# Rouslan/NTracer

Measured on AMD Instinct MI355X. Metric: Mrays/s (primary+shadow), 6-D hypercube @1920x1080, higher is better.
Workload: dtype f32

## Files before the change

ntracer_amd/csrc/nt_box.hpp:

```cpp
#pragma once
#include <type_traits>
#include "nt_pixel.hpp"

namespace {

__device__ __forceinline__ bool box_may_hit(int n, const float *dots, float sx, float sy, float sq) {
    const float osq = dots[0];
    const float ov = fmaf(-dots[2], sy, fmaf(dots[1], sx, dots[3]));
    const float rad2 = (float)n * (1.0f + NT_FUZZ) * (1.0f + NT_FUZZ) * 1.001f;
#ifdef NT_EXP_SKIP_SLABS
    return false;
#else
    return !((osq - rad2) * sq > ov * ov * 1.0001f);
#endif
}

__device__ __forceinline__ void box_background(float in, float &r, float &g, float &b) {
    if (in > 0.0f) { r = in; g = in; b = in; }
    else { r = 0.0f; g = -in; b = -in; }
}

template <int N>
__device__ __forceinline__ void box_color(const float (&o)[N], const float (&dir)[N], bool maybe, float &r, float &g, float &b) {
    bool done = false;
// ... 402 lines not shown
        return true;
    }
    emit_pixel(tg, pr, r, g, b);
    return true;
}

#ifndef NT_BOXROWS
#define NT_BOXROWS 8
#endif
template <int N>
__global__ __launch_bounds__(256) void box_kernel(NtCameraFixed cam, NtTarget tg) {
    const int tid = (int)threadIdx.x;
    float org[N], right[N], up[N], fwd[N], dir[N];
    load_camera<N>(cam, org, right, up, fwd);
    float margin = fabsf(org[0]);
#pragma unroll
    for (int j = 1; j < N; ++j) margin = fmaxf(margin, fabsf(org[j]));
    margin = NT_BOX_MARGIN * (1.0f + margin);
    float dots[4];
    if (cam.buf) {
        const float *dp = cam.dots + (size_t)blockIdx.z * 4;
        dots[0] = dp[0]; dots[1] = dp[1]; dots[2] = dp[2]; dots[3] = dp[3];
    } else {
        dots[0] = cam.odots[0]; dots[1] = cam.odots[1]; dots[2] = cam.odots[2]; dots[3] = cam.odots[3];
    }
    if (tg.colors_out) {
        const PixelRef pr = locate_pixel<64, 4>(tg, tid & 63, tid >> 6, tid);
        if (!pr.valid) return;
        const float sx = tg.fovI * ((float)pr.x - tg.half_w);
        const float sy = tg.fovI * ((float)pr.y - tg.half_h);
#pragma unroll
        for (int j = 0; j < N; ++j) dir[j] = (fwd[j] + right[j] * sx) - up[j] * sy;
        float sq = dir[0] * dir[0];
#pragma unroll
        for (int j = 1; j < N; ++j) sq = sq + dir[j] * dir[j];
        box_pixel<N, false>(tg, pr, org, dir, sq, dots, sx, sy, margin);
        return;
    }
    constexpr int R = NT_BOXROWS;
    const int row0 = ((int)blockIdx.y * 4 + __builtin_amdgcn_readfirstlane(tid >> 6)) * R;
    const int x = (int)blockIdx.x * 64 + (tid & 63);
    if (x >= tg.width) return;
    const float sx = tg.fovI * ((float)x - tg.half_w);
    float base[N];
#pragma unroll
    for (int j = 0; j < N; ++j) base[j] = fwd[j] + right[j] * sx;
    uint32_t live = ~0u;
    if (tg.cull) {
        if (row0 >= tg.row_count) return;
        const uint32_t *cp = tg.cull + ((size_t)blockIdx.z * tg.row_count + row0) * tg.cull_words + (blockIdx.x >> 3);
        live = 0u;
#pragma unroll
        for (int rr = 0; rr < R; ++rr) live |= (((cp[rr * tg.cull_words] >> (4 * (blockIdx.x & 7))) & 15u) != 0u ? 1u : 0u) << rr;
    }
    for (int rr = 0; rr < R; ++rr) {
        const int row = row0 + rr;
        if (row >= tg.row_count) return;
        const bool rowhit = (live >> rr) & 1u;
        const int orow = tg.row_begin + row;
        const int y = nt_image_row(tg, orow);
        if (y >= tg.height) continue;
        PixelRef pr;
        pr.x = x;
        pr.y = y;
        pr.offset = (long long)blockIdx.z * tg.frame_stride + (long long)(tg.compact ? orow : y) * tg.pitch + (long long)x * tg.bpp;
        pr.hit_index = 0;
        pr.valid = true;
        const float sy = tg.fovI * ((float)y - tg.half_h);
#pragma unroll
        for (int j = 0; j < N; ++j) dir[j] = base[j] - up[j] * sy;
        float sq = dir[0] * dir[0];
#pragma unroll
        for (int j = 1; j < N; ++j) sq = sq + dir[j] * dir[j];
        box_pixel<N, false>(tg, pr, org, dir, sq, dots, sx, sy, margin, rowhit);
    }
}

template <int N, int SPLIT>
__global__ __launch_bounds__(256) void box_redo_kernel(NtCameraFixed cam, NtTarget tg) {
    const int tid = (int)threadIdx.x;
    const int wv = __builtin_amdgcn_readfirstlane(tid >> 6);
    static_assert(SPLIT == 1 || SPLIT == 2 || SPLIT == 4, "waves per redo word");
    const int row = (int)blockIdx.y * (4 / SPLIT) + wv / SPLIT;
    if (row >= tg.row_count) return;
    uint32_t *word = tg.redo + ((size_t)blockIdx.z * tg.row_count + row) * tg.redo_words + blockIdx.x;
    const uint32_t mine = (SPLIT == 1 ? 0xffffffffu : SPLIT == 2 ? 0x55555555u : 0x11111111u) << (wv % SPLIT);
    uint32_t todo = *word & mine;
    if (todo == 0u) return;
    if ((tid & 63) == 0) {
        if (SPLIT > 1) atomicAnd(word, ~mine);
        else *word = 0u;
    }
    float org[N], right[N], up[N], fwd[N], dir[N];
    load_camera<N>(cam, org, right, up, fwd);
    float margin = fabsf(org[0]);
#pragma unroll
    for (int j = 1; j < N; ++j) margin = fmaxf(margin, fabsf(org[j]));
    margin = NT_BOX_MARGIN * (1.0f + margin);
    float dots[4];
    if (cam.buf) {
        const float *dp = cam.dots + (size_t)blockIdx.z * 4;
        dots[0] = dp[0]; dots[1] = dp[1]; dots[2] = dp[2]; dots[3] = dp[3];
    } else {
        dots[0] = cam.odots[0]; dots[1] = cam.odots[1]; dots[2] = cam.odots[2]; dots[3] = cam.odots[3];
    }
    const int orow = tg.row_begin + row;
    const int y = nt_image_row(tg, orow);
    if (y >= tg.height) return;
    const float sy = tg.fovI * ((float)y - tg.half_h);
    while (todo != 0u) {
        const int bit = __builtin_ctz(todo);
        todo &= todo - 1u;
        int x = ((int)blockIdx.x * 32 + bit) * 64 + (tid & 63);
        x = x < tg.width ? x : tg.width - 1;
        PixelRef pr;
        pr.x = x;
        pr.y = y;
        pr.offset = (long long)blockIdx.z * tg.frame_stride + (long long)(tg.compact ? orow : y) * tg.pitch + (long long)x * tg.bpp;
        pr.hit_index = 0;
        pr.valid = true;
        const float sx = tg.fovI * ((float)x - tg.half_w);
#pragma unroll
        for (int j = 0; j < N; ++j) dir[j] = (fwd[j] + right[j] * sx) - up[j] * sy;
        float sq = dir[0] * dir[0];
#pragma unroll
        for (int j = 1; j < N; ++j) sq = sq + dir[j] * dir[j];
        box_pixel<N, true, false, true>(tg, pr, org, dir, sq, dots, sx, sy, margin);
    }
}

template <int N, bool SETS = false>
__device__ __forceinline__ unsigned long long box_stretch_code2(const float (&org)[N], const float (&right)[N], const float (&up)[N],
                                                                const float (&fwd)[N], const NtTarget &tg, int y, int col) {
    uint32_t sets_value = 0u;
    uint32_t *const sets = SETS ? &sets_value : nullptr;
    uint32_t code = 0u;
    float omax = fabsf(org[0]);
#pragma unroll
    for (int j = 1; j < N; ++j) omax = fmaxf(omax, fabsf(org[j]));
    const float m = NT_BOX_MARGIN * (1.0f + omax);
    const float h = 1.0f + 2.0f * m + 1e-3f;
    const float sxc = tg.fovI * (((float)(col * 64) + 31.5f) - tg.half_w);
    const float sy = tg.fovI * ((float)y - tg.half_h);
    const float spread = 32.0f * tg.fovI;
    float tlo = 0.0f, thi = INFINITY;
    float vc[N], g[N];
    float tn = -INFINITY, tn2 = -INFINITY, vK = 0.0f, gK = 0.0f, oK = 0.0f;
    int K = 0;
#pragma unroll
    for (int j = 0; j < N; ++j) {
        vc[j] = (fwd[j] + right[j] * sxc) - up[j] * sy;
        g[j] = fmaf(spread, fabsf(right[j]), 1e-6f);
        const float pa = vc[j] + g[j], qa = -h - org[j];
        const float pb = vc[j] - g[j], qb = h - org[j];
        const float ra = qa * __builtin_amdgcn_rcpf(pa), rb = qb * __builtin_amdgcn_rcpf(pb);
        const bool ap = pa >= 0.0f, bp = pb >= 0.0f;
        const float lo_a = ap ? ra : -INFINITY, hi_a = ap ? INFINITY : ra;
        const float hi_b = bp ? rb : INFINITY, lo_b = bp ? -INFINITY : rb;
        tlo = nt_vmax3(tlo, lo_a, lo_b);
        thi = nt_vmin3(thi, hi_a, hi_b);
    }
    if (!(tlo > thi)) {
        code = 15u;
#pragma unroll
        for (int j = 0; j < N; ++j) {
            const float nr = ((vc[j] < 0.0f ? 1.0f : -1.0f) - org[j]) * __builtin_amdgcn_rcpf(vc[j]);
            tn2 = nt_vmed3(tn, tn2, nr);
            const bool later = nr > tn;
            vK = later ? vc[j] : vK;
            gK = later ? g[j] : gK;
            oK = later ? org[j] : oK;
            K = later ? j : K;
            tn = nt_vmax(tn, nr);
        }
        const float vKa = vK - gK, vKb = vK + gK;
        if (K < 13 && vKa * vKb > 0.0f) {
            const float num = (vK < 0.0f ? 1.0f : -1.0f) - oK;
            const float t1 = num * __builtin_amdgcn_rcpf(vKa), t2 = num * __builtin_amdgcn_rcpf(vKb);
            const float t_lo = nt_vmin(t1, t2) * (1.0f - 1e-6f), t_hi = nt_vmax(t1, t2) * (1.0f + 1e-6f);
            const float rK = m * __builtin_amdgcn_rcpf(fabsf(vK) - gK) * (1.0f + 1e-6f);
            bool ok = t_lo > 1e-3f && t_hi < 1e30f;
#pragma unroll
            for (int j = 0; j < N; ++j) {
                const float va = vc[j] - g[j], vb = vc[j] + g[j];
                const float pmax = org[j] + nt_vmax(vb * t_lo, vb * t_hi);
                const float pmin = org[j] + nt_vmin(va * t_lo, va * t_hi);
                const float lim = (1.0f - m - 1e-4f) - (fabsf(vc[j]) + g[j]) * rK;
                ok = ok && (j == K || (pmax <= lim && pmin >= -lim));
            }
            if (ok) code = (uint32_t)K + 1u;
        }
        if (code == 15u && !((tn - tn2) * fabsf(vK) > m)) code = 14u;
        if (code >= 14u) {
            if (sets != nullptr && N <= 10) {
                auto range = [&](int j, float &A, float &B, float &vabs) {
                    const float va = vc[j] - g[j], vb = vc[j] + g[j];
                    const float num = (vc[j] < 0.0f ? 1.0f : -1.0f) - org[j];
                    const float e1 = num * __builtin_amdgcn_rcpf(va), e2 = num * __builtin_amdgcn_rcpf(vb);
                    const float lo = nt_vmin(e1, e2), hi = nt_vmax(e1, e2);
                    const bool same = va * vb > 0.0f;
                    A = same ? lo - fabsf(lo) * 1e-6f : -INFINITY;
                    B = same ? hi + fabsf(hi) * 1e-6f : INFINITY;
                    vabs = same ? fabsf(vc[j]) - g[j] : 0.0f;
                };
                float rA[N], rB[N], rV[N];
                float TN = -INFINITY, TH = -INFINITY;
#pragma unroll
                for (int j = 0; j < N; ++j) {
                    range(j, rA[j], rB[j], rV[j]);
                    TN = nt_vmax(TN, rA[j]);
                    TH = nt_vmax(TH, rB[j]);
                }
                float vmin = INFINITY;
#pragma unroll
                for (int j = 0; j < N; ++j) vmin = rB[j] >= TN ? nt_vmin(vmin, rV[j]) : vmin;
                const float M = m * __builtin_amdgcn_rcpf(vmin) * (1.0f + 1e-5f);
                uint32_t T = 0u, C = 0u;
                float t_lo = INFINITY;
                const float t_hi = TH;
#pragma unroll
                for (int j = 0; j < N; ++j) {
                    const bool inT = rB[j] >= TN - M;
                    T |= inT ? 1u << j : 0u;
                    t_lo = inT ? nt_vmin(t_lo, rA[j]) : t_lo;
                }
#pragma unroll
                for (int j = 0; j < N; ++j) {
                    const float va = vc[j] - g[j], vb = vc[j] + g[j];
                    const float pmax = org[j] + nt_vmax(vb * t_lo, vb * t_hi);
                    const float pmin = org[j] + nt_vmin(va * t_lo, va * t_hi);
                    const float lim = 1.0f - m - 1e-4f;
                    const bool inC = ((T >> j) & 1u) != 0u || !(pmax <= lim && pmin >= -lim);
                    C |= inC ? 1u << j : 0u;
                }
                const bool valid = vmin > 0.0f && t_lo > 1e-3f && t_hi < 1e30f;
                *sets = valid ? (0x80000000u | (C << 10) | T) : 0u;
            }
        }
    }
    return (unsigned long long)code | ((unsigned long long)sets_value << 32);
}
template <int N>
__device__ __forceinline__ uint32_t box_stretch_code(const float (&org)[N], const float (&right)[N], const float (&up)[N], const float (&fwd)[N],
                                                     const NtTarget &tg, int y, int col) {
    return (uint32_t)box_stretch_code2<N, false>(org, right, up, fwd, tg, y, col);
}

template <int N>
__global__ __launch_bounds__(256) void box_cull_kernel(NtCameraFixed cam, NtTarget tg, uint32_t *out, int ncols) {
    float org[N], right[N], up[N], fwd[N];
    load_camera<N>(cam, org, right, up, fwd);
    const int word = (int)blockIdx.x, row = (int)blockIdx.y * 8 + (int)(threadIdx.x >> 5);
    const int col = word * 32 + (int)(threadIdx.x & 31);
    uint32_t code = 0u;
    if (row < tg.row_count && col < ncols) {
        const int orow = tg.row_begin + row;
        const int y = nt_image_row(tg, orow);
        code = box_stretch_code<N>(org, right, up, fwd, tg, y, col);
    }
    uint32_t packed = code << (4 * (threadIdx.x & 7));
    packed |= (uint32_t)__shfl_xor((int)packed, 1, 64);
    packed |= (uint32_t)__shfl_xor((int)packed, 2, 64);
    packed |= (uint32_t)__shfl_xor((int)packed, 4, 64);
    if (row < tg.row_count && (threadIdx.x & 7) == 0) out[((size_t)blockIdx.z * tg.row_count + row) * tg.cull_words + (col >> 3)] = packed;
}

#ifdef NT_EXP_NOSTORE
#define NT_EXP_STORE_IF if (tg.width < 0)
#else
#define NT_EXP_STORE_IF
#endif
#ifndef NT_TILE_OCC
#define NT_TILE_OCC
#endif
#ifndef NT_BOX_PIN_UP
#define NT_BOX_PIN_UP 1
#endif
#ifndef NT_BOX_LEAN_GROUPS_MAX_N
#define NT_BOX_LEAN_GROUPS_MAX_N 20
#endif
__device__ __forceinline__ bool guard_clear(float t) { return fabsf(__builtin_amdgcn_fractf(t) - 0.5f) > fmaf(t, 0x1p-18f, 0x1p-18f); }
__device__ __forceinline__ float lean_quotient(float d, float sy, float uu, float m2bu, float bb) {
    return fabsf(d) * __builtin_amdgcn_rsqf(fmaf(sy, fmaf(sy, uu, m2bu), bb));
}
template <int N>
__device__ __forceinline__ void pick_component(uint32_t K, const float (&base)[N], const float (&upv)[N], float &bK, float &uK) {
    bK = base[0];
    uK = upv[0];
#pragma unroll
    for (int j = 1; j < N; ++j) {
        bK = K == (uint32_t)j ? base[j] : bK;
        uK = K == (uint32_t)j ? upv[j] : uK;
    }
}
template <int N>
__device__ __forceinline__ float row_dir(const float (&base)[N], const float (&upv)[N], float sy, float (&dir)[N]) {
#pragma unroll
    for (int j = 0; j < N; ++j) dir[j] = base[j] - upv[j] * sy;
    float sq = dir[0] * dir[0];
#pragma unroll
    for (int j = 1; j < N; ++j) sq = sq + dir[j] * dir[j];
    return sq;
}
template <int N, bool F32, int ROWS, int WAVES>
__global__ __launch_bounds__(64 * WAVES) NT_TILE_OCC void box_tile_kernel(NtCameraFixed cam, NtTarget tg) {
    static_assert(ROWS == 8 || ROWS == 16 || ROWS == 32 || ROWS == 64, "sixteen row codes to a qword, one to four qwords a wave");
    static_assert(WAVES >= 1 && WAVES <= 4 && WAVES * ROWS <= 64, "the codes of a tile are the work of one wave, a row per lane");
    constexpr int R = ROWS;
    __shared__ uint32_t s_code[64];
    __shared__ unsigned long long s_rows[4];
    constexpr bool ALLIN = F32 || N <= NT_BOX_INLINE_MAX_N;
    constexpr bool SETS_LDS = ALLIN && N <= NT_BOX_SETS_MAX_N;
    __shared__ uint32_t s_sets[SETS_LDS ? 64 : 1];
    __shared__ int s_abort;
    const int tid = (int)threadIdx.x;
    const int lane = tid & 63;
    const int wv = __builtin_amdgcn_readfirstlane(tid >> 6);
#ifdef NT_EXP_TRACE
    const unsigned long long trace_t0 = wall_clock64();
    unsigned trace_rows = 0u;
    unsigned long long trace_t1 = 0ull;
#endif
    const unsigned nframes = gridDim.z - (unsigned)tg.lead_frames;
    unsigned frame = blockIdx.z;
    if (tg.lead_frames > 0) {
        const unsigned cols = gridDim.x, q = cols / 4u;
        const bool middle = blockIdx.x >= q && blockIdx.x < cols - q;
        if (!middle) frame -= (unsigned)tg.lead_frames;
        if (frame >= nframes) return;
    }
    float org[N], right[N], up[N], fwd[N], dir[N];
    load_camera<N>(cam, frame, org, right, up, fwd);
    float margin = fabsf(org[0]);
#pragma unroll
    for (int j = 1; j < N; ++j) margin = fmaxf(margin, fabsf(org[j]));
    margin = NT_BOX_MARGIN * (1.0f + margin);
    float dots[4];
    if (cam.buf) {
        const float *dp = cam.dots + (size_t)frame * 4;
        dots[0] = dp[0]; dots[1] = dp[1]; dots[2] = dp[2]; dots[3] = dp[3];
    } else {
        dots[0] = cam.odots[0]; dots[1] = cam.odots[1]; dots[2] = cam.odots[2]; dots[3] = cam.odots[3];
    }
    const int tile_row0 = (int)blockIdx.y * WAVES * R;
    if (wv == (int)((blockIdx.x + blockIdx.y + frame) % (unsigned)WAVES)) {
        if (tg.abort_word != nullptr) {
            const bool ab = nt_aborted(tg);
            if (WAVES == 1) { if (ab) return; }
            else if (lane == 0) s_abort = ab ? 1 : 0;
        }
        uint32_t code = 0u;
        uint32_t row_sets = 0u;
        const int trow = tg.row_il > 0 ? ((int)blockIdx.y * WAVES + lane / R) + tg.row_il * (lane % R) : tile_row0 + lane;
        if (lane < WAVES * R && trow < tg.row_count) {
            const int orow = tg.row_begin + trow;
            const int y = nt_image_row(tg, orow);
            if (y < tg.height) {
                const unsigned long long cs = box_stretch_code2<N, (N <= NT_BOX_SETS_MAX_N)>(org, right, up, fwd, tg, y, (int)blockIdx.x);
                code = (uint32_t)cs;
                row_sets = (uint32_t)(cs >> 32);
            }
        }
        if (SETS_LDS) s_sets[lane] = row_sets;
        {
            const unsigned long long m0 = __builtin_amdgcn_ballot_w64(code == 0u), m1 = __builtin_amdgcn_ballot_w64(code >= 1u && code <= 13u),
                                     m2 = __builtin_amdgcn_ballot_w64(code == 15u), m3 = __builtin_amdgcn_ballot_w64(code == 14u);
            if (lane == 0) {
                s_rows[0] = m0;
                s_rows[1] = m1;
                s_rows[2] = m2;
                s_rows[3] = m3;
            }
        }
        uint32_t packed = code << (4 * (lane & 7));
        packed |= (uint32_t)__shfl_xor((int)packed, 1, 64);
        packed |= (uint32_t)__shfl_xor((int)packed, 2, 64);
        packed |= (uint32_t)__shfl_xor((int)packed, 4, 64);
        if ((lane & 7) == 0) {
            const int grp = lane >> 3;
            const int slot = R == 8 ? 2 * grp : grp;
            s_code[slot] = packed;
            if (R == 8) s_code[slot + 1] = 0u;
        }
    }
    __syncthreads();
    if (WAVES > 1 && tg.abort_word != nullptr && s_abort != 0) return;
#ifdef NT_EXP_TRACE
    trace_t1 = wall_clock64();
#endif
    constexpr int HALVES = R >= 32 ? R / 16 : 1;
    const int wrow0 = tile_row0 + wv * R;
    const int il = tg.row_il;
    const int wfirst = il > 0 ? (int)blockIdx.y * WAVES + wv : wrow0;
    if (wfirst < tg.row_count) {
        typedef uint32_t nt_u32x4 __attribute__((ext_vector_type(4)));
        typedef __attribute__((address_space(4))) const nt_u32x4 *nt_rowtab;
        typedef uint32_t nt_u32x16 __attribute__((ext_vector_type(16), aligned(16)));
        typedef __attribute__((address_space(4))) const nt_u32x16 *nt_rowtab4;
        constexpr bool GROUPS = !F32 && N <= NT_BOX_LEAN_GROUPS_MAX_N;
        uint8_t *const frame_base = tg.dest + (long long)frame * tg.frame_stride;
#define NT_ROW_LOAD(rr)                     \
        const nt_u32x4 row_e = tab[(rr)];   \
        const float sy = __uint_as_float(row_e.x)
#define NT_ROW_OFF() ((long long)(((unsigned long long)row_e.w << 32) | row_e.z) + (long long)frame * tg.frame_stride)
#define NT_ROW_PTR() uniform_ptr(frame_base + (long long)(((unsigned long long)row_e.w << 32) | row_e.z))
#define NT_GROUP_PTR(k) uniform_ptr(frame_base + (long long)(((unsigned long long)grp_e[4 * (k) + 3] << 32) | grp_e[4 * (k) + 2]))
#define NT_LANE_OFF() ({ asm volatile("" : "+v"(xoff)); xoff; })
#define NT_CLEAR_BIT(mask, bit) asm("s_bitset0_b32 %0, %1" : "+s"(mask) : "s"(bit))
#define NT_SET_BIT(mask, bit) asm("s_bitset1_b32 %0, %1" : "+s"(mask) : "s"(bit))
        int x = (int)blockIdx.x * 64 + lane;
        x = x < tg.width ? x : tg.width - 1;
        uint32_t xoff = (uint32_t)x * (uint32_t)tg.bpp;
        const float sx = tg.fovI * ((float)x - tg.half_w);
        float base[N];
#pragma unroll
        for (int j = 0; j < N; ++j) base[j] = fwd[j] + right[j] * sx;
        float upv[N];
#pragma unroll
        for (int j = 0; j < N; ++j) {
            upv[j] = up[j];
            if (NT_BOX_PIN_UP || F32 || j == 0) asm volatile("" : "+v"(upv[j]));
        }
        float bb = 0.0f, bu = 0.0f, uu = 0.0f;
        bool fastsq = true;
        if (!F32) {
#pragma unroll
            for (int j = 0; j < N; ++j) {
                bb = fmaf(base[j], base[j], bb);
                bu = fmaf(base[j], up[j], bu);
                uu = fmaf(up[j], up[j], uu);
            }
            fastsq = __builtin_amdgcn_ballot_w64(!(bu * bu <= bb * uu * 0.0625f)) == 0ull;
        }
        const float maxv = (float)tg.plain_maxval;
        const float inv_maxv2 = 1.0f / (maxv * maxv);
        const float m2bu = (-2.0f * bu) * inv_maxv2;
        bb = bb * inv_maxv2;
        uu = uu * inv_maxv2;
        auto rows_of = [&](int k) {
            const unsigned long long m = s_rows[k];
            return (((unsigned long long)(uint32_t)__builtin_amdgcn_readfirstlane((int)(uint32_t)(m >> 32)) << 32) |
                    (uint32_t)__builtin_amdgcn_readfirstlane((int)(uint32_t)m)) >> (wv * R);
        };
        const unsigned long long rows_culled = rows_of(0), rows_face = rows_of(1), rows_rays = rows_of(2), rows_tie = rows_of(3);
        const int lrow = il > 0 ? wfirst + il * lane : wrow0 + lane;
        const int ly = nt_image_row(tg, tg.row_begin + lrow);
        const unsigned long long rows_valid = __builtin_amdgcn_ballot_w64(lane < R && lrow < tg.row_count && ly < tg.height);
#pragma unroll 1
        for (int half = 0; half < HALVES; ++half) {
        const int row0 = wrow0 + 16 * half;
        const int hfirst = il > 0 ? wfirst + il * 16 * half : row0;
        if (hfirst >= tg.row_count) break;
        uint32_t redo_bits = 0u;
        const int cw = (R >= 32 ? (R / 8) * wv + 2 * half : 2 * wv);
        unsigned long long rowcodes = ((unsigned long long)(uint32_t)__builtin_amdgcn_readfirstlane((int)s_code[cw + 1]) << 32) |
                                      (uint32_t)__builtin_amdgcn_readfirstlane((int)s_code[cw]);
        const uint32_t valid = HALVES > 1 ? (uint32_t)(rows_valid >> (16 * half)) & 0xffffu : (uint32_t)rows_valid;
        const nt_rowtab tab = (nt_rowtab)tg.rowtab + (il > 0 ? row0 : tg.row_begin + row0);
        uint32_t quick = (uint32_t)(rows_culled >> (16 * half)) & valid, inner = (uint32_t)(rows_face >> (16 * half)) & valid;
        uint32_t todo = (uint32_t)((ALLIN ? rows_rays | rows_tie : rows_rays) >> (16 * half)) & valid;
        if (!ALLIN) redo_bits = (uint32_t)(rows_tie >> (16 * half)) & valid;
#ifdef NT_EXP_TRACE
        trace_rows += (unsigned)__builtin_popcount(quick) | ((unsigned)__builtin_popcount(inner) << 8) |
                      ((unsigned)__builtin_popcount((uint32_t)(rows_rays >> (16 * half)) & valid) << 16) |
                      ((unsigned)__builtin_popcount((uint32_t)(rows_tie >> (16 * half)) & valid) << 24);
#endif
        if (!F32) {
            if (!fastsq) {
                todo |= quick | inner;
                quick = 0u;
                inner = 0u;
            }
            auto lean_rows = [&](auto sel8) {
            constexpr bool SEL8 = decltype(sel8)::value;
            auto put_quick = [&](nt_gptr out, float t, float d0) {
                if (SEL8) {
                    const uint32_t q = __float_as_uint(t + 8388608.0f);
                    NT_EXP_STORE_IF NT_G32(out) = __builtin_amdgcn_perm(d0 > 0.0f ? q : 0u, q, tg.plain_sel);
                    return;
                }
                uint32_t q = (uint32_t)(t + 0.5f);
                q = q < tg.plain_maxval ? q : tg.plain_maxval;
                const uint32_t w = (d0 > 0.0f ? q : 0u) * tg.plain_mul[0] + q * (tg.plain_mul[1] + tg.plain_mul[2]);
                NT_EXP_STORE_IF NT_G32(out) = tg.reversed ? w : bswap32(w);
            };
            auto put_face = [&](nt_gptr out, float t, float th) {
                if (SEL8) {
                    NT_EXP_STORE_IF NT_G32(out) = __builtin_amdgcn_perm(__float_as_uint(t + 8388608.0f), __float_as_uint(th + 8388608.0f), tg.plain_sel);
                    return;
                }
                uint32_t qr = (uint32_t)(t + 0.5f), qgb = (uint32_t)(th + 0.5f);
                qr = qr < tg.plain_maxval ? qr : tg.plain_maxval;
                qgb = qgb < tg.plain_maxval ? qgb : tg.plain_maxval;
                const uint32_t w = qr * tg.plain_mul[0] + qgb * (tg.plain_mul[1] + tg.plain_mul[2]);
                NT_EXP_STORE_IF NT_G32(out) = tg.reversed ? w : bswap32(w);
            };
            auto full_groups = [](uint32_t mask) { return mask & (mask >> 1) & (mask >> 2) & (mask >> 3) & 0x1111u; };
            auto lean_group = [&](int g, auto row, auto put) {
                const nt_u32x16 grp_e = *(nt_rowtab4)(tab + g);
                float a[4], b[4];
                unsigned long long fail[4];
#pragma unroll
                for (int k = 0; k < 4; ++k) fail[k] = __builtin_amdgcn_ballot_w64(!row(__uint_as_float(grp_e[4 * k]), a[k], b[k]));
                if (__builtin_expect(((fail[0] | fail[1]) | (fail[2] | fail[3])) == 0ull, 1)) {
                    const uint32_t xo = NT_LANE_OFF();
                    put(NT_GROUP_PTR(0) + xo, a[0], b[0]);
                    put(NT_GROUP_PTR(1) + xo, a[1], b[1]);
                    put(NT_GROUP_PTR(2) + xo, a[2], b[2]);
                    put(NT_GROUP_PTR(3) + xo, a[3], b[3]);
                } else {
                    todo |= ((fail[0] != 0ull ? 1u : 0u) | (fail[1] != 0ull ? 2u : 0u) | (fail[2] != 0ull ? 4u : 0u) | (fail[3] != 0ull ? 8u : 0u)) << g;
#pragma unroll
                    for (int k = 0; k < 4; ++k) {
                        if (fail[k] == 0ull) {
                            uint32_t xo = xoff;
                            asm volatile("" : "+v"(xo));
                            put(NT_GROUP_PTR(k) + xo, a[k], b[k]);
                        }
                    }
                }
            };
            auto culled_row = [&](float sy, float &t, float &d0) {
                d0 = base[0] - upv[0] * sy;
                t = lean_quotient(d0, sy, uu, m2bu, bb);
                return guard_clear(t);
            };
            auto face_row = [&](float bK, float uK, float sy, float &t, float &th) {
                const float dK = bK - uK * sy;
                t = lean_quotient(dK, sy, uu, m2bu, bb);
                th = t * 0.5f;
                return guard_clear(t) && guard_clear(th);
            };
            if (GROUPS) {
                uint32_t full = full_groups(quick);
                quick &= ~(full * 15u);
                while (full != 0u) {
                    const int g = __builtin_ctz(full);
                    NT_CLEAR_BIT(full, g);
                    lean_group(g, culled_row, put_quick);
                }
            }
            uint32_t quick_stored = 0u;
            for (uint32_t rest = quick; rest != 0u;) {
                const int rr = __builtin_ctz(rest);
                NT_CLEAR_BIT(rest, rr);
                NT_ROW_LOAD(rr);
                float t, d0;
                if (__builtin_expect(__builtin_amdgcn_ballot_w64(!culled_row(sy, t, d0)) == 0ull, 1)) {
                    put_quick(NT_ROW_PTR() + NT_LANE_OFF(), t, d0);
                    NT_SET_BIT(quick_stored, rr);
                }
            }
            todo |= quick & ~quick_stored;
            uint32_t K0 = 0u;
            float bK0 = base[0], uK0 = upv[0];
            if (inner != 0u) {
                K0 = ((uint32_t)(rowcodes >> (4 * __builtin_ctz(inner))) & 15u) - 1u;
                pick_component<N>(K0, base, upv, bK0, uK0);
            }
            if (GROUPS) {
                uint32_t full = full_groups(inner);
                const uint32_t same = (K0 + 1u) * 0x1111u;
                while (full != 0u) {
                    const int g = __builtin_ctz(full);
                    NT_CLEAR_BIT(full, g);
                    if (((uint32_t)(rowcodes >> (4 * g)) & 0xffffu) != same) continue;
                    inner &= ~(15u << g);
                    lean_group(g, [&](float sy, float &t, float &th) { return face_row(bK0, uK0, sy, t, th); }, put_face);
                }
            }
            uint32_t inner_stored = 0u;
            for (uint32_t rest = inner; rest != 0u;) {
                const int rr = __builtin_ctz(rest);
                NT_CLEAR_BIT(rest, rr);
                const uint32_t K = ((uint32_t)(rowcodes >> (4 * rr)) & 15u) - 1u;
                NT_ROW_LOAD(rr);
                float bK = bK0, uK = uK0;
                if (K != K0) pick_component<N>(K, base, upv, bK, uK);
                float t, th;
                if (__builtin_expect(__builtin_amdgcn_ballot_w64(!face_row(bK, uK, sy, t, th)) == 0ull, 1)) {
                    put_face(NT_ROW_PTR() + NT_LANE_OFF(), t, th);
                    NT_SET_BIT(inner_stored, rr);
                }
            }
            todo |= inner & ~inner_stored;
            };
            if (tg.plain_sel != 0u) lean_rows(std::true_type{});
            else lean_rows(std::false_type{});
        } else {
            while (quick != 0u) {
                const int rr = __builtin_ctz(quick);
                quick &= quick - 1u;
                NT_ROW_LOAD(rr);
                const float sq = row_dir<N>(base, upv, sy, dir);
                const float in = dir[0] / sqrt_wave(sq);
                float r, gb, b_;
                box_background(in, r, gb, b_);
                emit_f32x3_at(tg, NT_ROW_PTR() + NT_LANE_OFF(), r, gb);
            }
            uint32_t K0 = 0u;
            float bK0 = base[0], uK0 = upv[0];
            if (inner != 0u) {
                K0 = ((uint32_t)(rowcodes >> (4 * __builtin_ctz(inner))) & 15u) - 1u;
                pick_component<N>(K0, base, upv, bK0, uK0);
            }
            while (inner != 0u) {
                const int rr = __builtin_ctz(inner);
                inner &= inner - 1u;
                const uint32_t K = ((uint32_t)(rowcodes >> (4 * rr)) & 15u) - 1u;
                NT_ROW_LOAD(rr);
                const float sq = row_dir<N>(base, upv, sy, dir);
                float bK = bK0, uK = uK0;
                if (K != K0) pick_component<N>(K, base, upv, bK, uK);
                const float xk = bK - uK * sy;
                const float shade = fabsf(xk / sqrt_wave(sq));
                emit_f32x3_at(tg, NT_ROW_PTR() + NT_LANE_OFF(), shade * 1.0f, shade * 0.5f);
            }
        }
        while (todo != 0u) {
            const int rr = __builtin_ctz(todo);
            todo &= todo - 1u;
            const bool rowhit = ((uint32_t)(rowcodes >> (4 * rr)) & 15u) != 0u;
            NT_ROW_LOAD(rr);
            PixelRef pr;
            pr.x = x;
            pr.y = 0;
            pr.offset = NT_ROW_OFF() + (long long)xoff;
            pr.hit_index = 0;
            pr.valid = true;
            const float sq = row_dir<N>(base, upv, sy, dir);
            const int rcode = (int)((uint32_t)(rowcodes >> (4 * rr)) & 15u);
            if (ALLIN) {
                uint32_t sets = 0u;
                if (SETS_LDS) sets = (uint32_t)__builtin_amdgcn_readfirstlane((int)s_sets[wv * R + 16 * half + rr]);
                box_pixel<N, !F32, false, false, F32>(tg, pr, org, dir, sq, dots, sx, sy, margin, rowhit, rcode >= 1 && rcode <= 13 ? rcode - 1 : -1, sets,
                                                       rcode == 14);
            } else if (!box_pixel<N, true, true, false, false>(tg, pr, org, dir, sq, dots, sx, sy, margin, rowhit, rcode >= 1 && rcode <= 13 ? rcode - 1 : -1)) {
                redo_bits |= 1u << rr;
            }
        }
        if (!ALLIN && lane == 0) {
            while (redo_bits != 0u) {
                const int rr = __builtin_ctz(redo_bits);
                redo_bits &= redo_bits - 1u;
                const int mrow = il > 0 ? hfirst + il * rr : row0 + rr;
                atomicOr(tg.redo + ((size_t)frame * tg.row_count + mrow) * tg.redo_words + (blockIdx.x >> 5), 1u << (blockIdx.x & 31));
            }
        }
        }
    }
#ifdef NT_EXP_TRACE
    if (lane == 0) {
        unsigned long long *tr = reinterpret_cast<unsigned long long *>(tg.dest + (long long)nframes * tg.frame_stride) +
                                 ((((size_t)frame * gridDim.y + blockIdx.y) * gridDim.x + blockIdx.x) * WAVES + wv) * 4;
        tr[0] = trace_t0;
        tr[1] = wall_clock64();
        tr[2] = (unsigned long long)__builtin_amdgcn_s_getreg(4 | (31 << 11)) | ((unsigned long long)__builtin_amdgcn_s_getreg(20 | (31 << 11)) << 32);
        tr[3] = (unsigned long long)trace_rows | ((trace_t1 - trace_t0) << 32);
    }
#endif
#undef NT_ROW_LOAD
#undef NT_ROW_OFF
#undef NT_ROW_PTR
#undef NT_GROUP_PTR
#undef NT_LANE_OFF
#undef NT_CLEAR_BIT
#undef NT_SET_BIT
}

template <int N>
int launch_box_fixed(const NtLaunchInfo &li, const NtCamera &cam, const NtTarget &tg_in) {
    NtCameraFixed cf;
    cf.buf = cam.buf;
    cf.dots = cam.dots;
    for (int k = 0; k < 4; ++k) cf.odots[k] = cam.odots[k];
    cf.n = N;
    for (int k = 0; k < 4 * N; ++k) cf.inl[k] = cam.inl[k];
    NtTarget tg = tg_in;
    dim3 grid;
    grid_for(tg, 64, tg.colors_out ? 4 : 4 * NT_BOXROWS, li.nframes, grid);
    tg.cull = nullptr;
    tg.redo = nullptr;
    tg.cull_words = 0;
    tg.redo_words = 0;
    const bool fmt_rgb = tg.plain_bits != 0u && tg.plain_bits <= 10u && tg.bpp == 4 && tg.aligned4;
    const bool fmt_f32 = tg.plain_f32[0] >= 0 && tg.bpp == 12 && tg.aligned4;
    if (li.cull_buf && tg.rowtab && !tg.colors_out && (fmt_rgb || fmt_f32) && li.cull_clean) {
        hipStream_t st = (hipStream_t)li.stream;
        NtBoxTileGeom geom;
        geom.rows = li.tile_rows;
        geom.waves = li.tile_waves;
        const bool r64 = geom.rows == 64, r16 = geom.rows == 16;
        const int wpb = geom.waves;
        const int tile_rows = geom.rows * geom.waves;
        dim3 tgrid((unsigned)((tg.width + 63) / 64), (unsigned)((tg.row_count + tile_rows - 1) / tile_rows), (unsigned)li.nframes);
        tg.redo_words = ((tg.width + 63) / 64 + 31) / 32;
        tg.redo = li.cull_buf;
        tg.lead_frames = li.nframes >= 8 ? (li.nframes < 96 ? li.nframes : 96) : 0;
        if (tg.row_il > 0) tg.lead_frames = li.nframes >= 32 ? 16 : 0;
        if ((long long)li.nframes + tg.lead_frames > 65535) tg.lead_frames = 0;
        tgrid.z += (unsigned)tg.lead_frames;
        if (fmt_rgb) {
            if (r64) hipLaunchKernelGGL((box_tile_kernel<N, false, 64, 1>), tgrid, dim3(64), 0, st, cf, tg);
            else if (r16 && wpb == 3) hipLaunchKernelGGL((box_tile_kernel<N, false, 16, 3>), tgrid, dim3(192), 0, st, cf, tg);
            else if (r16) hipLaunchKernelGGL((box_tile_kernel<N, false, 16, 4>), tgrid, dim3(256), 0, st, cf, tg);
            else hipLaunchKernelGGL((box_tile_kernel<N, false, 8, 4>), tgrid, dim3(256), 0, st, cf, tg);
            if constexpr (N > NT_BOX_INLINE_MAX_N) {
                const long long rwords = (long long)tg.row_count * li.nframes * tg.redo_words;
                const int split = rwords < 48 * 1024 ? 2 : 1;
                const int rpb = 4 / split;
                const dim3 rgrid((unsigned)tg.redo_words, (unsigned)((tg.row_count + rpb - 1) / rpb), (unsigned)li.nframes);
                if (split == 2) hipLaunchKernelGGL((box_redo_kernel<N, 2>), rgrid, dim3(256), 0, st, cf, tg);
                else hipLaunchKernelGGL((box_redo_kernel<N, 1>), rgrid, dim3(256), 0, st, cf, tg);
            }
        } else {
            if (r64) hipLaunchKernelGGL((box_tile_kernel<N, true, 64, 1>), tgrid, dim3(64), 0, st, cf, tg);
            else if (r16 && wpb == 3) hipLaunchKernelGGL((box_tile_kernel<N, true, 16, 3>), tgrid, dim3(192), 0, st, cf, tg);
            else if (r16) hipLaunchKernelGGL((box_tile_kernel<N, true, 16, 4>), tgrid, dim3(256), 0, st, cf, tg);
            else hipLaunchKernelGGL((box_tile_kernel<N, true, 8, 4>), tgrid, dim3(256), 0, st, cf, tg);
        }
        return 0;
    }
    if (li.cull_buf && !tg.colors_out) {
        const int ncols = (tg.width + 63) / 64;
        const int words = (ncols + 31) / 32;
        tg.cull_words = 4 * words;
        hipLaunchKernelGGL(box_cull_kernel<N>, dim3((unsigned)words, (unsigned)((tg.row_count + 7) / 8), (unsigned)li.nframes), dim3(256), 0,
                           (hipStream_t)li.stream, cf, tg, li.cull_buf, ncols);
        tg.cull = li.cull_buf;
    }
    hipLaunchKernelGGL(box_kernel<N>, grid, dim3(256), 0, (hipStream_t)li.stream, cf, tg);
    return 0;
}

}
```

Before: 1.023 million.

## Keep per-row codes in registers for single-wave tiles and group face rows by axis

For single-wave blocks (ROWS=64), per-row codes and set bits now stay in a lane register and are read with readlane and ballots, instead of going through LDS with a block barrier. All 64 rows are handled in one pass using 64-bit masks. Face rows are grouped by hit axis, so each component is picked once per group and same-axis rows can use the grouped lean path. The cost is extra readlane traffic and 64-bit mask arithmetic. ROWS=32 configurations are no longer allowed.

After: 1.102 million, median of 6. 1.08x the previous value.

```diff
diff --git a/ntracer_amd/csrc/nt_box.hpp b/ntracer_amd/csrc/nt_box.hpp
--- a/ntracer_amd/csrc/nt_box.hpp
+++ b/ntracer_amd/csrc/nt_box.hpp
@@ -728,17 +728,34 @@
     for (int j = 1; j < N; ++j) sq = sq + dir[j] * dir[j];
     return sq;
 }
+#ifndef NT_BOX_PASS_ROWS
+#define NT_BOX_PASS_ROWS 64
+#endif
+__device__ __forceinline__ int nt_low_bit(uint32_t m) { return __builtin_ctz(m); }
+__device__ __forceinline__ int nt_low_bit(unsigned long long m) { return __builtin_ctzll(m); }
+__device__ __forceinline__ int nt_count_bits(uint32_t m) { return __builtin_popcount(m); }
+__device__ __forceinline__ int nt_count_bits(unsigned long long m) { return __builtin_popcountll(m); }
+__device__ __forceinline__ void nt_clear_bit(uint32_t &m, int bit) { asm("s_bitset0_b32 %0, %1" : "+s"(m) : "s"(bit)); }
+__device__ __forceinline__ void nt_clear_bit(unsigned long long &m, int bit) { asm("s_bitset0_b64 %0, %1" : "+s"(m) : "s"(bit)); }
+__device__ __forceinline__ void nt_set_bit(uint32_t &m, int bit) { asm("s_bitset1_b32 %0, %1" : "+s"(m) : "s"(bit)); }
+__device__ __forceinline__ void nt_set_bit(unsigned long long &m, int bit) { asm("s_bitset1_b64 %0, %1" : "+s"(m) : "s"(bit)); }
+__device__ __forceinline__ void nt_drop_low_bit(uint32_t &m, int) { m &= m - 1u; }
+__device__ __forceinline__ void nt_drop_low_bit(unsigned long long &m, int bit) { nt_clear_bit(m, bit); }
 template <int N, bool F32, int ROWS, int WAVES>
 __global__ __launch_bounds__(64 * WAVES) NT_TILE_OCC void box_tile_kernel(NtCameraFixed cam, NtTarget tg) {
-    static_assert(ROWS == 8 || ROWS == 16 || ROWS == 32 || ROWS == 64, "sixteen row codes to a qword, one to four qwords a wave");
+    static_assert(ROWS == 8 || ROWS == 16 || ROWS == 64, "a wave's rows: a qword of sixteen codes in LDS or fewer, or one row a lane");
     static_assert(WAVES >= 1 && WAVES <= 4 && WAVES * ROWS <= 64, "the codes of a tile are the work of one wave, a row per lane");
+    static_assert(WAVES == 1 ? ROWS == 64 : ROWS <= 16, "one wave a block renders the 64 rows whose codes it worked out itself");
     constexpr int R = ROWS;
-    __shared__ uint32_t s_code[64];
-    __shared__ unsigned long long s_rows[4];
+    constexpr bool REG = WAVES == 1;
+    constexpr int LDS_N = REG ? 1 : 64;
+    __shared__ uint32_t s_code[LDS_N];
+    __shared__ unsigned long long s_rows[REG ? 1 : 4];
     constexpr bool ALLIN = F32 || N <= NT_BOX_INLINE_MAX_N;
     constexpr bool SETS_LDS = ALLIN && N <= NT_BOX_SETS_MAX_N;
-    __shared__ uint32_t s_sets[SETS_LDS ? 64 : 1];
+    __shared__ uint32_t s_sets[SETS_LDS ? LDS_N : 1];
     __shared__ int s_abort;
+    uint32_t lane_cs = 0u;
     const int tid = (int)threadIdx.x;
     const int lane = tid & 63;
     const int wv = __builtin_amdgcn_readfirstlane(tid >> 6);
@@ -769,11 +786,11 @@
         dots[0] = cam.odots[0]; dots[1] = cam.odots[1]; dots[2] = cam.odots[2]; dots[3] = cam.odots[3];
     }
     const int tile_row0 = (int)blockIdx.y * WAVES * R;
-    if (wv == (int)((blockIdx.x + blockIdx.y + frame) % (unsigned)WAVES)) {
+    if (REG || wv == (int)((blockIdx.x + blockIdx.y + frame) % (unsigned)WAVES)) {
         if (tg.abort_word != nullptr) {
             const bool ab = nt_aborted(tg);
-            if (WAVES == 1) { if (ab) return; }
-            else if (lane == 0) s_abort = ab ? 1 : 0;
+            if constexpr (REG) { if (ab) return; }
+            else { if (lane == 0) s_abort = ab ? 1 : 0; }
         }
         uint32_t code = 0u;
         uint32_t row_sets = 0u;
@@ -787,34 +804,42 @@
                 row_sets = (uint32_t)(cs >> 32);
             }
         }
-        if (SETS_LDS) s_sets[lane] = row_sets;
-        {
-            const unsigned long long m0 = __builtin_amdgcn_ballot_w64(code == 0u), m1 = __builtin_amdgcn_ballot_w64(code >= 1u && code <= 13u),
-                                     m2 = __builtin_amdgcn_ballot_w64(code == 15u), m3 = __builtin_amdgcn_ballot_w64(code == 14u);
-            if (lane == 0) {
-                s_rows[0] = m0;
-                s_rows[1] = m1;
-                s_rows[2] = m2;
-                s_rows[3] = m3;
-            }
-        }
-        uint32_t packed = code << (4 * (lane & 7));
-        packed |= (uint32_t)__shfl_xor((int)packed, 1, 64);
-        packed |= (uint32_t)__shfl_xor((int)packed, 2, 64);
-        packed |= (uint32_t)__shfl_xor((int)packed, 4, 64);
-        if ((lane & 7) == 0) {
-            const int grp = lane >> 3;
-            const int slot = R == 8 ? 2 * grp : grp;
-            s_code[slot] = packed;
-            if (R == 8) s_code[slot + 1] = 0u;
-        }
-    }
-    __syncthreads();
-    if (WAVES > 1 && tg.abort_word != nullptr && s_abort != 0) return;
+        if constexpr (REG) {
+            lane_cs = (SETS_LDS ? row_sets & 0x800fffffu : 0u) | (code << 20);
+        } else {
+            if (SETS_LDS) s_sets[lane] = row_sets;
+            {
+                const unsigned long long m0 = __builtin_amdgcn_ballot_w64(code == 0u), m1 = __builtin_amdgcn_ballot_w64(code >= 1u && code <= 13u),
+                                         m2 = __builtin_amdgcn_ballot_w64(code == 15u), m3 = __builtin_amdgcn_ballot_w64(code == 14u);
+                if (lane == 0) {
+                    s_rows[0] = m0;
+                    s_rows[1] = m1;
+                    s_rows[2] = m2;
+                    s_rows[3] = m3;
+                }
+            }
+            uint32_t packed = code << (4 * (lane & 7));
+            packed |= (uint32_t)__shfl_xor((int)packed, 1, 64);
+            packed |= (uint32_t)__shfl_xor((int)packed, 2, 64);
+            packed |= (uint32_t)__shfl_xor((int)packed, 4, 64);
+            if ((lane & 7) == 0) {
+                const int grp = lane >> 3;
+                const int slot = R == 8 ? 2 * grp : grp;
+                s_code[slot] = packed;
+                if (R == 8) s_code[slot + 1] = 0u;
+            }
+        }
+    }
+    if constexpr (!REG) {
+        __syncthreads();
+        if (tg.abort_word != nullptr && s_abort != 0) return;
+    }
 #ifdef NT_EXP_TRACE
     trace_t1 = wall_clock64();
 #endif
-    constexpr int HALVES = R >= 32 ? R / 16 : 1;
+    constexpr int PASS = R == 64 ? NT_BOX_PASS_ROWS : R;
+    static_assert(PASS == R || (R == 64 && PASS == 16), "NT_BOX_PASS_ROWS: 64 or 16");
+    typedef typename std::conditional<PASS == 64, unsigned long long, uint32_t>::type mask_t;
     const int wrow0 = tile_row0 + wv * R;
     const int il = tg.row_il;
     const int wfirst = il > 0 ? (int)blockIdx.y * WAVES + wv : wrow0;
@@ -832,8 +857,8 @@
 #define NT_ROW_PTR() uniform_ptr(frame_base + (long long)(((unsigned long long)row_e.w << 32) | row_e.z))
 #define NT_GROUP_PTR(k) uniform_ptr(frame_base + (long long)(((unsigned long long)grp_e[4 * (k) + 3] << 32) | grp_e[4 * (k) + 2]))
 #define NT_LANE_OFF() ({ asm volatile("" : "+v"(xoff)); xoff; })
-#define NT_CLEAR_BIT(mask, bit) asm("s_bitset0_b32 %0, %1" : "+s"(mask) : "s"(bit))
-#define NT_SET_BIT(mask, bit) asm("s_bitset1_b32 %0, %1" : "+s"(mask) : "s"(bit))
+#define NT_CLEAR_BIT(mask, bit) nt_clear_bit(mask, bit)
+#define NT_SET_BIT(mask, bit) nt_set_bit(mask, bit)
         int x = (int)blockIdx.x * 64 + lane;
         x = x < tg.width ? x : tg.width - 1;
         uint32_t xoff = (uint32_t)x * (uint32_t)tg.bpp;
@@ -863,33 +888,62 @@
         const float m2bu = (-2.0f * bu) * inv_maxv2;
         bb = bb * inv_maxv2;
         uu = uu * inv_maxv2;
-        auto rows_of = [&](int k) {
-            const unsigned long long m = s_rows[k];
-            return (((unsigned long long)(uint32_t)__builtin_amdgcn_readfirstlane((int)(uint32_t)(m >> 32)) << 32) |
-                    (uint32_t)__builtin_amdgcn_readfirstlane((int)(uint32_t)m)) >> (wv * R);
-        };
-        const unsigned long long rows_culled = rows_of(0), rows_face = rows_of(1), rows_rays = rows_of(2), rows_tie = rows_of(3);
+        const uint32_t lane_code = (lane_cs >> 20) & 15u;
+        unsigned long long rows_culled, rows_face, rows_rays, rows_tie;
+        if constexpr (REG) {
+            rows_culled = __builtin_amdgcn_ballot_w64(lane_code == 0u);
+            rows_face = __builtin_amdgcn_ballot_w64(lane_code >= 1u && lane_code <= 13u);
+            rows_rays = __builtin_amdgcn_ballot_w64(lane_code == 15u);
+            rows_tie = __builtin_amdgcn_ballot_w64(lane_code == 14u);
+        } else {
+            auto rows_of = [&](int k) {
+                const unsigned long long m = s_rows[k];
+                return (((unsigned long long)(uint32_t)__builtin_amdgcn_readfirstlane((int)(uint32_t)(m >> 32)) << 32) |
+                        (uint32_t)__builtin_amdgcn_readfirstlane((int)(uint32_t)m)) >> (wv * R);
+            };
+            rows_culled = rows_of(0);
+            rows_face = rows_of(1);
+            rows_rays = rows_of(2);
+            rows_tie = rows_of(3);
+        }
         const int lrow = il > 0 ? wfirst + il * lane : wrow0 + lane;
         const int ly = nt_image_row(tg, tg.row_begin + lrow);
         const unsigned long long rows_valid = __builtin_amdgcn_ballot_w64(lane < R && lrow < tg.row_count && ly < tg.height);
 #pragma unroll 1
-        for (int half = 0; half < HALVES; ++half) {
-        const int row0 = wrow0 + 16 * half;
-        const int hfirst = il > 0 ? wfirst + il * 16 * half : row0;
+        for (int pass = 0; pass < R / PASS; ++pass) {
+        const int slot0 = PASS * pass;
+        const int row0 = wrow0 + slot0;
+        const int hfirst = il > 0 ? wfirst + il * slot0 : row0;
         if (hfirst >= tg.row_count) break;
-        uint32_t redo_bits = 0u;
-        const int cw = (R >= 32 ? (R / 8) * wv + 2 * half : 2 * wv);
-        unsigned long long rowcodes = ((unsigned long long)(uint32_t)__builtin_amdgcn_readfirstlane((int)s_code[cw + 1]) << 32) |
-                                      (uint32_t)__builtin_amdgcn_readfirstlane((int)s_code[cw]);
-        const uint32_t valid = HALVES > 1 ? (uint32_t)(rows_valid >> (16 * half)) & 0xffffu : (uint32_t)rows_valid;
+        mask_t redo_bits = 0u;
+        unsigned long long rowcodes = 0ull;
+        if constexpr (!REG) {
+            rowcodes = ((unsigned long long)(uint32_t)__builtin_amdgcn_readfirstlane((int)s_code[2 * wv + 1]) << 32) |
+                       (uint32_t)__builtin_amdgcn_readfirstlane((int)s_code[2 * wv]);
+        }
+        auto slot_word = [&](int rr) { return (uint32_t)__builtin_amdgcn_readlane((int)lane_cs, slot0 + rr); };
+        auto code_of = [&](int rr) {
+            if constexpr (REG) return (slot_word(rr) >> 20) & 15u;
+            else return (uint32_t)(rowcodes >> (4 * rr)) & 15u;
+        };
+        auto sets_of = [&](int rr) {
+            if constexpr (!SETS_LDS) return 0u;
+            else if constexpr (REG) return slot_word(rr) & 0x800fffffu;
+            else return (uint32_t)__builtin_amdgcn_readfirstlane((int)s_sets[wv * R + rr]);
+        };
+        auto rows_with_code = [&](uint32_t c) {
+            if constexpr (REG) return (mask_t)(__builtin_amdgcn_ballot_w64(lane_code == c) >> slot0);
+            else return (mask_t)__builtin_amdgcn_ballot_w64(lane < PASS && ((uint32_t)(rowcodes >> (4 * (lane & 15))) & 15u) == c);
+        };
+        const mask_t valid = R > PASS ? (mask_t)(rows_valid >> slot0) & (mask_t)((1ull << (PASS & 63)) - 1ull) : (mask_t)rows_valid;
         const nt_rowtab tab = (nt_rowtab)tg.rowtab + (il > 0 ? row0 : tg.row_begin + row0);
-        uint32_t quick = (uint32_t)(rows_culled >> (16 * half)) & valid, inner = (uint32_t)(rows_face >> (16 * half)) & valid;
-        uint32_t todo = (uint32_t)((ALLIN ? rows_rays | rows_tie : rows_rays) >> (16 * half)) & valid;
-        if (!ALLIN) redo_bits = (uint32_t)(rows_tie >> (16 * half)) & valid;
+        mask_t quick = (mask_t)(rows_culled >> slot0) & valid, inner = (mask_t)(rows_face >> slot0) & valid;
+        mask_t todo = (mask_t)((ALLIN ? rows_rays | rows_tie : rows_rays) >> slot0) & valid;
+        if (!ALLIN) redo_bits = (mask_t)(rows_tie >> slot0) & valid;
 #ifdef NT_EXP_TRACE
-        trace_rows += (unsigned)__builtin_popcount(quick) | ((unsigned)__builtin_popcount(inner) << 8) |
-                      ((unsigned)__builtin_popcount((uint32_t)(rows_rays >> (16 * half)) & valid) << 16) |
-                      ((unsigned)__builtin_popcount((uint32_t)(rows_tie >> (16 * half)) & valid) << 24);
+        trace_rows += (unsigned)nt_count_bits(quick) | ((unsigned)nt_count_bits(inner) << 8) |
+                      ((unsigned)nt_count_bits((mask_t)(rows_rays >> slot0) & valid) << 16) |
+                      ((unsigned)nt_count_bits((mask_t)(rows_tie >> slot0) & valid) << 24);
 #endif
         if (!F32) {
             if (!fastsq) {
@@ -899,15 +953,20 @@
             }
             auto lean_rows = [&](auto sel8) {
             constexpr bool SEL8 = decltype(sel8)::value;
+#ifdef NT_EXP_RED_BY_SHIFT
+#define NT_RED_OF(q, d0) ((q) & (uint32_t)((int32_t)__float_as_uint(d0) >> 31))
+#else
+#define NT_RED_OF(q, d0) ((d0) > 0.0f ? (q) : 0u)
+#endif
             auto put_quick = [&](nt_gptr out, float t, float d0) {
                 if (SEL8) {
                     const uint32_t q = __float_as_uint(t + 8388608.0f);
-                    NT_EXP_STORE_IF NT_G32(out) = __builtin_amdgcn_perm(d0 > 0.0f ? q : 0u, q, tg.plain_sel);
+                    NT_EXP_STORE_IF NT_G32(out) = __builtin_amdgcn_perm(NT_RED_OF(q, d0), q, tg.plain_sel);
                     return;
                 }
                 uint32_t q = (uint32_t)(t + 0.5f);
                 q = q < tg.plain_maxval ? q : tg.plain_maxval;
-                const uint32_t w = (d0 > 0.0f ? q : 0u) * tg.plain_mul[0] + q * (tg.plain_mul[1] + tg.plain_mul[2]);
+                const uint32_t w = NT_RED_OF(q, d0) * tg.plain_mul[0] + q * (tg.plain_mul[1] + tg.plain_mul[2]);
                 NT_EXP_STORE_IF NT_G32(out) = tg.reversed ? w : bswap32(w);
             };
             auto put_face = [&](nt_gptr out, float t, float th) {
@@ -921,7 +980,7 @@
                 const uint32_t w = qr * tg.plain_mul[0] + qgb * (tg.plain_mul[1] + tg.plain_mul[2]);
                 NT_EXP_STORE_IF NT_G32(out) = tg.reversed ? w : bswap32(w);
             };
-            auto full_groups = [](uint32_t mask) { return mask & (mask >> 1) & (mask >> 2) & (mask >> 3) & 0x1111u; };
+            auto full_groups = [](mask_t mask) { return mask & (mask >> 1) & (mask >> 2) & (mask >> 3) & (mask_t)(PASS == 64 ? 0x1111111111111111ull : 0x1111ull); };
             auto lean_group = [&](int g, auto row, auto put) {
                 const nt_u32x16 grp_e = *(nt_rowtab4)(tab + g);
                 float a[4], b[4];
@@ -935,7 +994,7 @@
                     put(NT_GROUP_PTR(2) + xo, a[2], b[2]);
                     put(NT_GROUP_PTR(3) + xo, a[3], b[3]);
                 } else {
-                    todo |= ((fail[0] != 0ull ? 1u : 0u) | (fail[1] != 0ull ? 2u : 0u) | (fail[2] != 0ull ? 4u : 0u) | (fail[3] != 0ull ? 8u : 0u)) << g;
+                    todo |= (mask_t)((fail[0] != 0ull ? 1u : 0u) | (fail[1] != 0ull ? 2u : 0u) | (fail[2] != 0ull ? 4u : 0u) | (fail[3] != 0ull ? 8u : 0u)) << g;
 #pragma unroll
                     for (int k = 0; k < 4; ++k) {
                         if (fail[k] == 0ull) {
@@ -947,7 +1006,11 @@
                 }
             };
             auto culled_row = [&](float sy, float &t, float &d0) {
+#ifdef NT_EXP_RED_BY_SHIFT
+                d0 = upv[0] * sy - base[0];
+#else
                 d0 = base[0] - upv[0] * sy;
+#endif
                 t = lean_quotient(d0, sy, uu, m2bu, bb);
                 return guard_clear(t);
             };
@@ -958,17 +1021,17 @@
                 return guard_clear(t) && guard_clear(th);
             };
             if (GROUPS) {
-                uint32_t full = full_groups(quick);
+                mask_t full = full_groups(quick);
                 quick &= ~(full * 15u);
                 while (full != 0u) {
-                    const int g = __builtin_ctz(full);
+                    const int g = nt_low_bit(full);
                     NT_CLEAR_BIT(full, g);
                     lean_group(g, culled_row, put_quick);
                 }
             }
-            uint32_t quick_stored = 0u;
-            for (uint32_t rest = quick; rest != 0u;) {
-                const int rr = __builtin_ctz(rest);
+            mask_t quick_stored = 0u;
+            for (mask_t rest = quick; rest != 0u;) {
+                const int rr = nt_low_bit(rest);
                 NT_CLEAR_BIT(rest, rr);
                 NT_ROW_LOAD(rr);
                 float t, d0;
@@ -978,45 +1041,41 @@
                 }
             }
             todo |= quick & ~quick_stored;
-            uint32_t K0 = 0u;
-            float bK0 = base[0], uK0 = upv[0];
-            if (inner != 0u) {
-                K0 = ((uint32_t)(rowcodes >> (4 * __builtin_ctz(inner))) & 15u) - 1u;
-                pick_component<N>(K0, base, upv, bK0, uK0);
-            }
-            if (GROUPS) {
-                uint32_t full = full_groups(inner);
-                const uint32_t same = (K0 + 1u) * 0x1111u;
-                while (full != 0u) {
-                    const int g = __builtin_ctz(full);
-                    NT_CLEAR_BIT(full, g);
-                    if (((uint32_t)(rowcodes >> (4 * g)) & 0xffffu) != same) continue;
-                    inner &= ~(15u << g);
-                    lean_group(g, [&](float sy, float &t, float &th) { return face_row(bK0, uK0, sy, t, th); }, put_face);
-                }
-            }
-            uint32_t inner_stored = 0u;
-            for (uint32_t rest = inner; rest != 0u;) {
-                const int rr = __builtin_ctz(rest);
-                NT_CLEAR_BIT(rest, rr);
-                const uint32_t K = ((uint32_t)(rowcodes >> (4 * rr)) & 15u) - 1u;
-                NT_ROW_LOAD(rr);
-                float bK = bK0, uK = uK0;
-                if (K != K0) pick_component<N>(K, base, upv, bK, uK);
-                float t, th;
-                if (__builtin_expect(__builtin_amdgcn_ballot_w64(!face_row(bK, uK, sy, t, th)) == 0ull, 1)) {
-                    put_face(NT_ROW_PTR() + NT_LANE_OFF(), t, th);
-                    NT_SET_BIT(inner_stored, rr);
-                }
-            }
-            todo |= inner & ~inner_stored;
+            while (inner != 0u) {
+                const uint32_t code0 = code_of(nt_low_bit(inner));
+                float bK0, uK0;
+                pick_component<N>(code0 - 1u, base, upv, bK0, uK0);
+                mask_t same = inner & rows_with_code(code0);
+                inner &= ~same;
+                if (GROUPS) {
+                    mask_t full = full_groups(same);
+                    same &= ~(full * 15u);
+                    while (full != 0u) {
+                        const int g = nt_low_bit(full);
+                        NT_CLEAR_BIT(full, g);
+                        lean_group(g, [&](float sy, float &t, float &th) { return face_row(bK0, uK0, sy, t, th); }, put_face);
+                    }
+                }
+                mask_t same_stored = 0u;
+                for (mask_t rest = same; rest != 0u;) {
+                    const int rr = nt_low_bit(rest);
+                    NT_CLEAR_BIT(rest, rr);
+                    NT_ROW_LOAD(rr);
+                    float t, th;
+                    if (__builtin_expect(__builtin_amdgcn_ballot_w64(!face_row(bK0, uK0, sy, t, th)) == 0ull, 1)) {
+                        put_face(NT_ROW_PTR() + NT_LANE_OFF(), t, th);
+                        NT_SET_BIT(same_stored, rr);
+                    }
+                }
+                todo |= same & ~same_stored;
+            }
             };
             if (tg.plain_sel != 0u) lean_rows(std::true_type{});
             else lean_rows(std::false_type{});
         } else {
             while (quick != 0u) {
-                const int rr = __builtin_ctz(quick);
-                quick &= quick - 1u;
+                const int rr = nt_low_bit(quick);
+                nt_drop_low_bit(quick, rr);
                 NT_ROW_LOAD(rr);
                 const float sq = row_dir<N>(base, upv, sy, dir);
                 const float in = dir[0] / sqrt_wave(sq);
@@ -1024,29 +1083,28 @@
                 box_background(in, r, gb, b_);
                 emit_f32x3_at(tg, NT_ROW_PTR() + NT_LANE_OFF(), r, gb);
             }
-            uint32_t K0 = 0u;
-            float bK0 = base[0], uK0 = upv[0];
-            if (inner != 0u) {
-                K0 = ((uint32_t)(rowcodes >> (4 * __builtin_ctz(inner))) & 15u) - 1u;
-                pick_component<N>(K0, base, upv, bK0, uK0);
-            }
             while (inner != 0u) {
-                const int rr = __builtin_ctz(inner);
-                inner &= inner - 1u;
-                const uint32_t K = ((uint32_t)(rowcodes >> (4 * rr)) & 15u) - 1u;
-                NT_ROW_LOAD(rr);
-                const float sq = row_dir<N>(base, upv, sy, dir);
-                float bK = bK0, uK = uK0;
-                if (K != K0) pick_component<N>(K, base, upv, bK, uK);
-                const float xk = bK - uK * sy;
-                const float shade = fabsf(xk / sqrt_wave(sq));
-                emit_f32x3_at(tg, NT_ROW_PTR() + NT_LANE_OFF(), shade * 1.0f, shade * 0.5f);
+                const uint32_t code0 = code_of(nt_low_bit(inner));
+                float bK0, uK0;
+                pick_component<N>(code0 - 1u, base, upv, bK0, uK0);
+                mask_t same = inner & rows_with_code(code0);
+                inner &= ~same;
+                while (same != 0u) {
+                    const int rr = nt_low_bit(same);
+                    nt_drop_low_bit(same, rr);
+                    NT_ROW_LOAD(rr);
+                    const float sq = row_dir<N>(base, upv, sy, dir);
+                    const float xk = bK0 - uK0 * sy;
+                    const float shade = fabsf(xk / sqrt_wave(sq));
+                    emit_f32x3_at(tg, NT_ROW_PTR() + NT_LANE_OFF(), shade * 1.0f, shade * 0.5f);
+                }
             }
         }
         while (todo != 0u) {
-            const int rr = __builtin_ctz(todo);
-            todo &= todo - 1u;
-            const bool rowhit = ((uint32_t)(rowcodes >> (4 * rr)) & 15u) != 0u;
+            const int rr = nt_low_bit(todo);
+            nt_drop_low_bit(todo, rr);
+            const int rcode = (int)code_of(rr);
+            const bool rowhit = rcode != 0;
             NT_ROW_LOAD(rr);
             PixelRef pr;
             pr.x = x;
@@ -1055,20 +1113,17 @@
             pr.hit_index = 0;
             pr.valid = true;
             const float sq = row_dir<N>(base, upv, sy, dir);
-            const int rcode = (int)((uint32_t)(rowcodes >> (4 * rr)) & 15u);
             if (ALLIN) {
-                uint32_t sets = 0u;
-                if (SETS_LDS) sets = (uint32_t)__builtin_amdgcn_readfirstlane((int)s_sets[wv * R + 16 * half + rr]);
-                box_pixel<N, !F32, false, false, F32>(tg, pr, org, dir, sq, dots, sx, sy, margin, rowhit, rcode >= 1 && rcode <= 13 ? rcode - 1 : -1, sets,
-                                                       rcode == 14);
+                box_pixel<N, !F32, false, false, F32>(tg, pr, org, dir, sq, dots, sx, sy, margin, rowhit, rcode >= 1 && rcode <= 13 ? rcode - 1 : -1,
+                                                       sets_of(rr), rcode == 14);
             } else if (!box_pixel<N, true, true, false, false>(tg, pr, org, dir, sq, dots, sx, sy, margin, rowhit, rcode >= 1 && rcode <= 13 ? rcode - 1 : -1)) {
-                redo_bits |= 1u << rr;
+                redo_bits |= (mask_t)1u << rr;
             }
         }
         if (!ALLIN && lane == 0) {
             while (redo_bits != 0u) {
-                const int rr = __builtin_ctz(redo_bits);
-                redo_bits &= redo_bits - 1u;
+                const int rr = nt_low_bit(redo_bits);
+                nt_drop_low_bit(redo_bits, rr);
                 const int mrow = il > 0 ? hfirst + il * rr : row0 + rr;
                 atomicOr(tg.redo + ((size_t)frame * tg.row_count + mrow) * tg.redo_words + (blockIdx.x >> 5), 1u << (blockIdx.x & 31));
             }
@@ -1092,6 +1147,7 @@
 #undef NT_LANE_OFF
 #undef NT_CLEAR_BIT
 #undef NT_SET_BIT
+#undef NT_RED_OF
 }
 
 template <int N>
```
